# wbw520/scouter

Measured on AMD Instinct MI355X. Metric: images/sec training step (resnest26d+xSlot, 224^2, bs70), higher is better.
Workload: dtype f32; 1 GPU; BASELINE configs[1]: ImageNet-10 resnest26d + positive xSlot, channel 2048, T=3, to_k_layer 3, power 2, 224x224, per-GPU batch 70, random init, AdamW lr 1e-4; precision=fp32, activation_storage=fp32, register_split_bf16x3_layers=16, global_batch=70, parallelism=dp1, step=zero_grad+fwd+loss+bwd(+allreduce)+adamw, launch=eager

## Files before the change

### include/scouter_hip.h

```cpp
#ifndef SCOUTER_HIP_H
#define SCOUTER_HIP_H
#include <stddef.h>
#ifdef __cplusplus
extern "C" {
#endif

#define SC_OK 0
#define SC_ERR_ARG (-1)
#define SC_ERR_LAUNCH (-2)
#define SC_ERR_UNSUPPORTED (-3)
#define SC_ERR_WORKSPACE (-4)

int scouter_abi_version(void);
const char* scouter_last_error(void);

int scouter_set_switch(const char* name, int value);
int scouter_get_switch(const char* name);

int scouter_resize_normalize_u8_f32(const unsigned char* const* srcs, const int* hw, unsigned char* tmp,
                                    const long* tmp_off, const float* lut, float* out, int B, int C, int max_h, int max_w,
                                    int out_h, int out_w, void* stream);

void scouter_prof_enable(int on);
int scouter_prof_collect(char* buf, int cap);
// ... 258 lines not shown

int scouter_linear_small_fwd_f32(const float* x, const float* w, const float* bias, float* y, int B, int K, int C,
                                 void* stream);
int scouter_linear_small_bwd_f32(const float* dy, const float* x, const float* w, float* dx, float* dw, float* db,
                                 int B, int K, int C, void* stream);

int scouter_planes_split_f32(const float* x, void* planes, long n, int nplanes, void* stream);
int scouter_planes_split_weight_f32(const float* w_hwio, void* w_fwd, void* w_dgrad, int kh, int kw, int Cin, int Cout,
                                    int groups, int nplanes, void* stream);
size_t scouter_planes_split_weights_row_bytes(void);
int scouter_planes_split_weights_multi(const void* table, int nrows, long total, int nplanes, void* stream);
int scouter_conv2d_fwd_planes_bn_partial_rows(int B, int H, int W, int kh, int kw, int stride, int pad);
int scouter_conv2d_fwd_planes_io(const void* x_planes, const void* w_planes, const float* bias, const float* addend,
                                 void* y, double* bn_partial, int B, int H, int W, int Cin, int Cout, int kh, int kw,
                                 int stride, int pad, int groups, int relu, int nplanes, int tile, int io, void* stream);
int scouter_conv2d_fwd_planes(const void* x_planes, const void* w_planes, const float* bias, const float* addend,
                              float* y, double* bn_partial, int B, int H, int W, int Cin, int Cout, int kh, int kw,
                              int stride, int pad, int groups, int relu, int nplanes, int tile, void* stream);
int scouter_conv2d_dgrad_planes(const void* dy_planes, const void* w_planes, const float* addend, float* dx, int B, int H,
                                int W, int Cin, int Cout, int kh, int kw, int stride, int pad, int groups, int nplanes,
                                int tile, void* stream);
int scouter_conv2d_dgrad_planes_bnbwd(const void* dy_planes, const void* w_planes, const float* addend, float* dx, int B,
                                      int H, int W, int Cin, int Cout, int kh, int kw, int stride, int pad, int groups,
                                      int nplanes, int tile, const void* relu_mask, const float* x1,
                                      const float* saved1, double* part1, const float* x2, const float* saved2,
                                      double* part2, void* stream);

size_t scouter_conv2d_wgrad_planes_workspace_bytes(int B, int H, int W, int Cin, int Cout, int kh, int kw, int groups,
                                                   int plan_hint);
int scouter_conv2d_wgrad_planes(const void* x_planes, const void* dy_planes, float* dw, int B, int H, int W, int Cin,
                                int Cout, int kh, int kw, int pad, int groups, int nplanes, int plan_hint,
                                void* ws, size_t ws_bytes, void* stream);

int scouter_conv2d_x3_tile(long M, int N, int tile_hint);
int scouter_conv2d_x3_partial_rows(long M, int N, int tile_hint);
int scouter_conv2d_x3_halo_partial_rows(int groups);
int scouter_conv2d_fwd_x3(const float* x, const void* w_planes_fwd, const float* bias, const float* addend, float* y,
                          double* bn_partial, int B, int H, int W, int Cin, int Cout, int kh, int kw, int pad, int groups,
                          int relu, int tile_hint, void* stream);
int scouter_conv2d_dgrad_x3_bnbwd(const float* dy, const void* w_planes_dgrad, const float* addend, float* dx, int B,
                                  int H, int W, int Cin, int Cout, int kh, int kw, int pad, int groups, int tile_hint,
                                  const void* relu_mask, const float* x1, const float* saved1, double* part1,
                                  const float* x2, const float* saved2, double* part2, void* stream);

size_t scouter_conv2d_wgrad_x3_workspace_bytes(int B, int H, int W, int Cin, int Cout, int plan_hint);
int scouter_conv2d_wgrad_x3(const float* x, const float* dy, float* dw, int B, int H, int W, int Cin, int Cout,
                            int plan_hint, void* ws, size_t ws_bytes, void* stream);

size_t scouter_bn_fold_row_bytes(void);
int scouter_bn_fold_multi(const void* table, int nrows, long total, void* stream);
int scouter_sa_gate_fwd_f32(const float* gap, const float* w1, const float* b1, const float* w2, const float* b2, float* a,
                            int B, int Cp, int A, void* stream);

int scouter_iadd_i64(long* p, long n, long v, void* stream);

int scouter_adamw_chunk_bytes(void);
int scouter_adamw_step_f32(const void* chunk_table, int nchunks, const float* grads, float* exp_avg,
                           float* exp_avg_sq, float lr, float beta1, float beta2, float eps, float weight_decay,
                           int step, void* stream);
int scouter_adamw_step_dev_f32(const void* chunk_table, int nchunks, const float* grads, float* exp_avg,
                               float* exp_avg_sq, const float* dyn, float beta1, float beta2, float eps,
                               float weight_decay, void* stream);

#ifdef __cplusplus
}
#endif
#endif
```

### scouter_amd/csrc/abi_core.hip

```cpp
#include "common.h"

#include <stdarg.h>
#include <stdlib.h>
#include <atomic>
#include <map>
#include <mutex>
#include <vector>

#define SCOUTER_ABI_VERSION 1

static thread_local char g_err[512] = "";
static thread_local hipError_t g_lds_err = hipSuccess;

void sc_set_error(const char* fmt, ...) {
    va_list ap;
    va_start(ap, fmt);
    vsnprintf(g_err, sizeof(g_err), fmt, ap);
    va_end(ap);
}

int sc_check_launch(const char* what) {
    hipError_t e = hipGetLastError();
    if (e == hipSuccess) e = g_lds_err;
    g_lds_err = hipSuccess;
    if (e != hipSuccess) {
        sc_set_error("%s: launch failed: %s", what, hipGetErrorString(e));
        return SC_ERR_LAUNCH;
    }
    return SC_OK;
}

extern "C" int scouter_abi_version(void) { return SCOUTER_ABI_VERSION; }
extern "C" const char* scouter_last_error(void) { return g_err; }

static const char* const g_switch_names[SC_SW_COUNT] = {"xwt", "bwt", "bhalo", "xslot_small", "xslot_bwd_halves",
                                                         "xslot_bwd_scratch", "pwp_bn", "pwp_resident"};
struct SwitchTable {
    std::atomic<int> v[SC_SW_COUNT] = {};
    SwitchTable() {
        static const char* const flags[] = {"SCOUTER_XWT", "SCOUTER_BWT", "SCOUTER_BHALO", "SCOUTER_XSLOT_SMALL",
                                            "SCOUTER_XSLOT_BWD_HALVES", "SCOUTER_XSLOT_BWD_SCRATCH"};
        for (int i = 0; i <= SC_SW_XSLOT_BWD_SCRATCH; ++i) {
            const int def = i != SC_SW_XSLOT_BWD_SCRATCH;
            const char* e = getenv(flags[i]);
            v[i] = e && e[0] == '1' - def ? !def : def;
        }
        int bn = 0, r = 0;
        const char* e = getenv("SCOUTER_PWP_PLAN_DEV");
        if (e && sscanf(e, "%d,%d", &bn, &r) == 2 && bn > 0 && r > 0) { v[SC_SW_PWP_BN] = bn; v[SC_SW_PWP_RESIDENT] = r; }
    }
};
static SwitchTable& switch_table() {
    static SwitchTable t;
    return t;
}
int sc_switch(ScSwitch s) { return switch_table().v[s].load(std::memory_order_relaxed); }

static int switch_index(const char* name) {
    for (int i = 0; name && i < SC_SW_COUNT; ++i)
        if (strcmp(name, g_switch_names[i]) == 0) return i;
    sc_set_error("unknown switch '%s'", name ? name : "(null)");
    return -1;
}
extern "C" int scouter_set_switch(const char* name, int value) {
    const int i = switch_index(name);
    if (i < 0) return SC_ERR_ARG;
    SC_REQUIRE(value >= 0, "switch '%s': negative value %d", name, value);
    switch_table().v[i].store(value, std::memory_order_relaxed);
    return SC_OK;
}
extern "C" int scouter_get_switch(const char* name) {
    const int i = switch_index(name);
    return i < 0 ? SC_ERR_ARG : sc_switch((ScSwitch)i);
}

void sc_dyn_lds(const void* kern, size_t bytes) {
    static std::mutex mu;
    static std::map<std::pair<const void*, int>, size_t> limits;
    int dev = 0;
    hipGetDevice(&dev);
    std::lock_guard<std::mutex> lk(mu);
    size_t& have = limits[{kern, dev}];
    if (bytes <= have) return;
    const hipError_t e = hipFuncSetAttribute(kern, hipFuncAttributeMaxDynamicSharedMemorySize, (int)bytes);
    if (e == hipSuccess) have = bytes;
    else g_lds_err = e;
}

struct ProfRec { hipEvent_t a, b; const char* name; double flops, bytes; };
static std::mutex g_prof_mu;
static bool g_prof_on = false;
static std::vector<ProfRec> g_prof;

ScProfScope::ScProfScope(const char* name, hipStream_t st, double flops, double bytes) : stream(st), slot(-1) {
    if (!g_prof_on) return;
// ... 47 lines not shown
```

### scouter_amd/csrc/common.h

```cpp
#pragma once
#include <hip/hip_runtime.h>
#include <stdint.h>
#include <stdio.h>
#include <string.h>

#define SC_OK 0
#define SC_ERR_ARG (-1)
#define SC_ERR_LAUNCH (-2)
#define SC_ERR_UNSUPPORTED (-3)
#define SC_ERR_WORKSPACE (-4)

typedef float f32x4 __attribute__((ext_vector_type(4)));
typedef float f32x16 __attribute__((ext_vector_type(16)));

void sc_set_error(const char* fmt, ...);
int sc_check_launch(const char* what);

enum ScSwitch { SC_SW_XWT, SC_SW_BWT, SC_SW_BHALO, SC_SW_XSLOT_SMALL, SC_SW_XSLOT_BWD_HALVES, SC_SW_XSLOT_BWD_SCRATCH,
                SC_SW_PWP_BN, SC_SW_PWP_RESIDENT, SC_SW_COUNT };
int sc_switch(ScSwitch s);

void sc_dyn_lds(const void* kern, size_t bytes);

#define SC_REQUIRE(cond, ...)                 \
    do {                                      \
        if (!(cond)) {                        \
            sc_set_error(__VA_ARGS__);        \
            return SC_ERR_ARG;                \
        }                                     \
    } while (0)

#define SC_UNSUPPORTED(cond, ...)             \
    do {                                      \
        if (!(cond)) {                        \
            sc_set_error(__VA_ARGS__);        \
            return SC_ERR_UNSUPPORTED;        \
        }                                     \
    } while (0)

struct ScProfScope {
    hipStream_t stream;
    int slot;
    ScProfScope(const char* name, hipStream_t stream, double flops, double bytes);
    ~ScProfScope();
};

static inline int sc_cdiv(long a, long b) { return (int)((a + b - 1) / b); }

__device__ __forceinline__ f32x16 mfma32(float a, float b, f32x16 c) {
    return __builtin_amdgcn_mfma_f32_32x32x2f32(a, b, c, 0, 0, 0);
}
__device__ __forceinline__ int mfma32_row(int reg, int lane) { return (reg & 3) + 8 * (reg >> 2) + 4 * (lane >> 5); }

__device__ __forceinline__ float wave_sum(float v) {
#pragma unroll
    for (int o = 32; o > 0; o >>= 1) v += __shfl_xor(v, o, 64);
    return v;
}
__device__ __forceinline__ double wave_sum_d(double v) {
#pragma unroll
    for (int o = 32; o > 0; o >>= 1) v += __shfl_xor(v, o, 64);
    return v;
}

typedef unsigned short u16x4 __attribute__((ext_vector_type(4)));
__device__ __forceinline__ void split3_bf16(float x, unsigned short& h, unsigned short& m, unsigned short& l) {
    const __bf16 bh = (__bf16)x;
    const float r1 = x - (float)bh;
    const __bf16 bm = (__bf16)r1;
    const float r2 = r1 - (float)bm;
    const __bf16 bl = (__bf16)r2;
    h = __builtin_bit_cast(unsigned short, bh);
// ... 122 lines not shown
```

### scouter_amd/kernels.py

```python
import contextlib
import os
import sys
import types

import torch

from . import _native

F32 = torch.float32
BF16 = torch.bfloat16
IO_X_BF16, IO_Y_BF16, IO_R_BF16 = 1, 2, 4
DGRAD_IO_ADDEND, DGRAD_IO_DY, DGRAD_IO_DX = 4, 8, 16
_ws = {}


_raw_stream = getattr(torch._C, "_cuda_getCurrentRawStream", None)


def _stream():
    if _raw_stream is not None:
        return _raw_stream(torch.cuda.current_device())
    return torch.cuda.current_stream().cuda_stream


# ... 1078 lines not shown
    ws = _sa_ws(B, H * W, C2, x.device)
    _native.check(_native.lib().scouter_sa_reduce_io(_p(x), _p(dout), _p(bn), _p(out), _p(sums), B, H * W, C2 // 2, 1,
                                                     IO_X_BF16 if x.dtype == BF16 else 0, _p(ws), ws.numel(), _stream()),
                  "sa_dattn")
    return (out, sums) if want_stats else out


def sa_bn_bwd(dout, a, dgap, x0, bn, training, dgamma=None, dbeta=None, planes=0, keep_f32=True, sums=None):
    _chk(x0, "x0", (F32, BF16)); _chk(dout, "dout")
    B, H, W, Cp = dout.shape
    dx = torch.empty(x0.shape, dtype=F32, device=x0.device) if keep_f32 or not planes else None
    dxp = torch.empty((planes,) + tuple(x0.shape), dtype=BF16, device=x0.device) if planes else None
    ws = _col_ws(B * H * W, 2 * Cp, x0.device)
    _native.check(_native.lib().scouter_sa_bn_bwd_io(_p(dout), _p(a), _p(dgap), _p(x0), _p(bn), _p(sums), B, H * W, Cp,
                                                     int(training), _p(dgamma), _p(dbeta), _p(dx), _p(dxp), planes,
                                                     IO_X_BF16 if x0.dtype == BF16 else 0, _p(ws), ws.numel(), _stream()),
                  "sa_bn_bwd")
    return PlaneTensor(dx, dxp) if planes else dx


def radix_softmax_fwd(z):
    a = torch.empty_like(z)
    _native.check(_native.lib().scouter_radix_softmax_fwd_f32(_p(z), _p(a), z.shape[0], z.shape[1] // 2, _stream()),
                  "radix_softmax_fwd")
    return a


def radix_softmax_bwd(a, da):
    dz = torch.empty_like(a)
    _native.check(_native.lib().scouter_radix_softmax_bwd_f32(_p(a), _p(da), _p(dz), a.shape[0], a.shape[1] // 2,
                                                              _stream()), "radix_softmax_bwd")
    return dz


SA_GATE_THREADS = 256


def sa_gate_eligible(Cp, A):
    return A in (32, 64, 128, 256) and Cp <= 512 and Cp % (8 * (SA_GATE_THREADS // A)) == 0


def sa_gate_fwd(gap, w1, b1, w2, b2):
    for n, t in (("gap", gap), ("w1", w1), ("b1", b1), ("w2", w2), ("b2", b2)):
        _chk(t, n)
    B, Cp = gap.shape
    A = w1.shape[-1]
    assert tuple(w1.shape[-2:]) == (Cp, A) and tuple(w2.shape[-2:]) == (A, 2 * Cp) and b1.numel() == A and b2.numel() == 2 * Cp
    a = torch.empty((B, 2 * Cp), dtype=F32, device=gap.device)
    _native.check(_native.lib().scouter_sa_gate_fwd_f32(_p(gap), _p(w1), _p(b1), _p(w2), _p(b2), _p(a), B, Cp, A, _stream()),
                  "sa_gate_fwd")
    return a


class BnFolder:

    def __init__(self, items):
        import struct
        L = _native.lib()
        dev = items[0][0].device
        self.key = self.pointers(items)
        if any(it[0].data_ptr() % 16 for it in items):
            raise RuntimeError("scouter_amd: the one-launch fold reads the weights as 16-byte vectors: unaligned weight storage")
        al = lambda n: (n + 63) // 64 * 64
        offs, off = [], 0
        for w, cb, g, be, mu, var, eps, rows_pad in items:
            cout = w.shape[-1]
            rows = w.numel() // cout
            if cout % 4 or rows_pad and rows_pad < rows:
                raise RuntimeError("scouter_amd: the one-launch fold takes 4-multiples of output channels, got %s" % (tuple(w.shape),))
            offs.append((off, off + al(max(rows, rows_pad) * cout)))
            off = offs[-1][1] + al(cout)
        self.flat = torch.zeros(off, dtype=F32, device=dev)
        rows_blob, self.outs, first = [], [], 0
        for (w, cb, g, be, mu, var, eps, rows_pad), (ow, ob) in zip(items, offs):
            for n, t in (("weight", w), ("conv bias", cb), ("gamma", g), ("beta", be), ("running_mean", mu), ("running_var", var)):
                _chk(t, n)
            cout = w.shape[-1]
            rows = w.numel() // cout
            shape = (1, 1, rows_pad, cout) if rows_pad else tuple(w.shape)
            wo = self.flat[ow:ow + max(rows, rows_pad) * cout].view(shape)
            bo = self.flat[ob:ob + cout]
            rows_blob.append(struct.pack("<6Qd2Qiiq", w.data_ptr(), _p(cb) or 0, g.data_ptr(), be.data_ptr(), mu.data_ptr(),
                                         var.data_ptr(), float(eps), wo.data_ptr(), bo.data_ptr(), rows, cout, first))
            self.outs.append((wo, bo))
            first += rows * cout
        blob = b"".join(rows_blob)
        assert len(blob) == len(items) * L.scouter_bn_fold_row_bytes()
        self.table = torch.frombuffer(bytearray(blob), dtype=torch.uint8).to(dev)
        self.total = first

    @staticmethod
    def pointers(items):
        return tuple(t.data_ptr() if t is not None else 0 for it in items for t in it[:6])

    def run(self):
        _native.check(_native.lib().scouter_bn_fold_multi(_p(self.table), len(self.outs), self.total, _stream()), "bn_fold_multi")
        return self.outs


def sa_apply_fwd(x, a, bn=None, out_dtype=F32):
    _chk(x, "x", (F32, BF16))
    B, H, W, C2 = x.shape
    out = torch.empty((B, H, W, C2 // 2), dtype=out_dtype, device=x.device)
    _native.check(_native.lib().scouter_sa_apply_fwd_io(
        _p(x), _p(a), _p(bn), _p(out), B, H * W, C2 // 2,
        (IO_X_BF16 if x.dtype == BF16 else 0) | (IO_Y_BF16 if out_dtype == BF16 else 0), _stream()), "sa_apply_fwd")
# ... 696 lines not shown
```

### scouter_amd/timm/models/layers/split_attn.py

```python
import os

import torch.nn as nn

from ....nn_hip import Act, BatchNorm2d, Conv2d
from .... import kernels as K

SA_SUMS = os.environ.get("SCOUTER_SA_SUMS", "1") == "1"


class SplitAttnConv2d(nn.Module):
    def __init__(self, in_channels, out_channels, kernel_size=3, stride=1, padding=1, groups=1, radix=2,
                 reduction_factor=4):
        super().__init__()
        if radix != 2 or groups != 1:
            raise NotImplementedError("scouter_amd supports the radix-2 / cardinality-1 split attention of "
                                      "resnest26d / resnest50d only")
        self.radix = radix
        mid_chs = out_channels * radix
        attn_chs = max(in_channels * radix // reduction_factor, 32)
        self.conv = Conv2d(in_channels, mid_chs, kernel_size, stride, padding, groups=groups * radix, bias=False)
        self.bn0 = BatchNorm2d(mid_chs)
        self.act0 = Act()
        self.fc1 = Conv2d(out_channels, attn_chs, 1, bias=True)
        self.bn1 = BatchNorm2d(attn_chs)
        self.act1 = Act()
        self.fc2 = Conv2d(attn_chs, mid_chs, 1, bias=True)

    def fwd(self, x, save, tracked=None, x0_dtype=None, out_dtype=None):
        c, c_conv = self.conv.fwd(x, save, bn_stats=self.bn0.training, out_dtype=x0_dtype)
        x0, saved0 = self.bn0.stats_only(c, tracked)
        B = x0.shape[0]
        gap = K.sa_gap(x0, saved0)
        z1, c_fc1 = self.fc1.fwd(gap.view(B, 1, 1, -1), save, bn_stats=self.bn1.training)
        g1, c_bn1 = self.bn1.fwd(z1, save, relu=True, tracked=tracked)
        z2, c_fc2 = self.fc2.fwd(g1, save)
        a = K.radix_softmax_fwd(z2.view(B, -1))
        out = K.sa_apply_fwd(x0, a, saved0, out_dtype=out_dtype or K.F32)
        return out, ((c_conv, x0, saved0, self.bn0.training, c_fc1, c_bn1, c_fc2, a) if save else None)

    def fwd_folded(self, x):
        x0 = self.conv.fwd_folded(x, relu=True)
        B = x0.shape[0]
        gap = K.sa_gap(x0, None)
        if K.sa_gate_eligible(gap.shape[1], self.fc1.out_channels):
            f = self.fc1._fold
            a = K.sa_gate_fwd(gap, f.w, f.b, K.hwio(self.fc2.weight), self.fc2.bias)
        else:
            g1 = self.fc1.fwd_folded(gap.view(B, 1, 1, -1), relu=True)
            z2, _ = self.fc2.fwd(g1, False)
            a = K.radix_softmax_fwd(z2.view(B, -1))
        return K.sa_apply_fwd(x0, a, None)

    def bwd(self, dout, ctx, post=None):
        c_conv, x0, saved0, training0, c_fc1, c_bn1, c_fc2, a = ctx
        B = x0.shape[0]
        da, sums = K.sa_dattn(x0, dout, saved0, want_stats=True) if SA_SUMS else (K.sa_dattn(x0, dout, saved0), None)
        dz2 = K.radix_softmax_bwd(a, da)
        dg1 = self.fc2.bwd(dz2.view(B, 1, 1, -1), c_fc2, True)
        dz1, _ = self.bn1.bwd(dg1, c_bn1)
        dgap = self.fc1.bwd(dz1, c_fc1, True)
        on_planes = c_conv.wd is not None
        only = on_planes and c_conv.xp is not None and self.conv.planes_only(x0.shape[1], x0.shape[2])
        planes = self.conv.route().planes_dy if on_planes else 0
        if not planes and self.conv.dy_plane_only(*x0.shape[:3]):
            planes, only = 1, True
        dc = K.sa_bn_bwd(dout, a, dgap.view(B, -1), x0, saved0, training0, self.bn0._dg, self.bn0._db,
                         planes=planes, keep_f32=not only, sums=sums)
        return self.conv.bwd(dc, c_conv, True, post=post)
```

Before: 4819 images/sec.

## Fuse split-attention gate fc1+BN+ReLU, fc2+softmax and backward into custom kernels

Adds dedicated HIP kernels for the split-attention gate in training: fc1 with batch-norm stats and ReLU, fc2 with radix softmax, a fused softmax-backward/fc2-dgrad/BN-backward kernel, an fc1 dgrad kernel, and a combined weight-gradient kernel that runs on a side stream. The aim is to replace a chain of many small launches (conv, BN, softmax, colsum) on tiny B x C tensors with a few launches. The path is gated by a new default-on switch and a shape eligibility check. The trade-off is added code complexity and a different numerical path for BN statistics, which are accumulated in double.

```diff
diff --git a/include/scouter_hip.h b/include/scouter_hip.h
--- a/include/scouter_hip.h
+++ b/include/scouter_hip.h
@@ -334,6 +334,20 @@
 int scouter_sa_gate_fwd_f32(const float* gap, const float* w1, const float* b1, const float* w2, const float* b2, float* a,
                             int B, int Cp, int A, void* stream);
 
+int scouter_sa_gate_train_ok(int B, int Cp, int A);
+int scouter_sa_gate_train_max_batch(void);
+int scouter_sa_gate_fc1_bn_f32(const float* gap, const float* w1, const float* b1, const float* gamma, const float* beta,
+                               float* running_mean, float* running_var, float momentum, float eps, float* z1, float* g1,
+                               float* saved, int B, int Cp, int A, void* stream);
+int scouter_sa_gate_fc2_softmax_f32(const float* g1, const float* w2, const float* b2, float* a, int B, int Cp, int A,
+                                    void* stream);
+int scouter_sa_gate_bwd_fc2_bn_f32(const float* a, const float* da, const float* w2, const float* g1, const float* z1,
+                                   const float* gamma, float eps, float* dz2, float* dz1, float* dgamma, float* dbeta, int B,
+                                   int Cp, int A, void* stream);
+int scouter_sa_gate_bwd_fc1_f32(const float* dz1, const float* w1, float* dgap, int B, int Cp, int A, void* stream);
+int scouter_sa_gate_wgrad_f32(const float* gap, const float* dz1, const float* g1, const float* dz2, float* dw1, float* db1,
+                              float* dw2, float* db2, int B, int Cp, int A, void* stream);
+
 int scouter_iadd_i64(long* p, long n, long v, void* stream);
 
 int scouter_adamw_chunk_bytes(void);
diff --git a/scouter_amd/csrc/abi_core.hip b/scouter_amd/csrc/abi_core.hip
--- a/scouter_amd/csrc/abi_core.hip
+++ b/scouter_amd/csrc/abi_core.hip
@@ -34,13 +34,13 @@
 extern "C" const char* scouter_last_error(void) { return g_err; }
 
 static const char* const g_switch_names[SC_SW_COUNT] = {"xwt", "bwt", "bhalo", "xslot_small", "xslot_bwd_halves",
-                                                         "xslot_bwd_scratch", "pwp_bn", "pwp_resident"};
+                                                         "xslot_bwd_scratch", "sa_gate_train", "pwp_bn", "pwp_resident"};
 struct SwitchTable {
     std::atomic<int> v[SC_SW_COUNT] = {};
     SwitchTable() {
         static const char* const flags[] = {"SCOUTER_XWT", "SCOUTER_BWT", "SCOUTER_BHALO", "SCOUTER_XSLOT_SMALL",
-                                            "SCOUTER_XSLOT_BWD_HALVES", "SCOUTER_XSLOT_BWD_SCRATCH"};
-        for (int i = 0; i <= SC_SW_XSLOT_BWD_SCRATCH; ++i) {
+                                            "SCOUTER_XSLOT_BWD_HALVES", "SCOUTER_XSLOT_BWD_SCRATCH", "SCOUTER_SA_GATE_TRAIN"};
+        for (int i = 0; i <= SC_SW_SA_GATE_TRAIN; ++i) {
             const int def = i != SC_SW_XSLOT_BWD_SCRATCH;
             const char* e = getenv(flags[i]);
             v[i] = e && e[0] == '1' - def ? !def : def;
diff --git a/scouter_amd/csrc/common.h b/scouter_amd/csrc/common.h
--- a/scouter_amd/csrc/common.h
+++ b/scouter_amd/csrc/common.h
@@ -17,7 +17,7 @@
 int sc_check_launch(const char* what);
 
 enum ScSwitch { SC_SW_XWT, SC_SW_BWT, SC_SW_BHALO, SC_SW_XSLOT_SMALL, SC_SW_XSLOT_BWD_HALVES, SC_SW_XSLOT_BWD_SCRATCH,
-                SC_SW_PWP_BN, SC_SW_PWP_RESIDENT, SC_SW_COUNT };
+                SC_SW_SA_GATE_TRAIN, SC_SW_PWP_BN, SC_SW_PWP_RESIDENT, SC_SW_COUNT };
 int sc_switch(ScSwitch s);
 
 void sc_dyn_lds(const void* kern, size_t bytes);
diff --git a/scouter_amd/csrc/sa_gate_train.hip b/scouter_amd/csrc/sa_gate_train.hip
--- /dev/null
+++ b/scouter_amd/csrc/sa_gate_train.hip
@@ -0,0 +1,391 @@
+#include "common.h"
+
+#define SGT_THREADS 256
+#define SGT_MAX_B 256
+#define SGT_MAX_CP 512
+#define SGT_MAX_A 256
+#define SGT_NC 8
+#ifndef SGT_FC1_ACC
+#define SGT_FC1_ACC double
+#endif
+
+static bool sgt_shape_ok(long B, long Cp, long A) {
+    return (A == 32 || A == 64 || A == 128 || A == 256) && Cp >= 32 && Cp <= SGT_MAX_CP && Cp % 32 == 0 && B >= 2 &&
+           B <= SGT_MAX_B;
+}
+extern "C" int scouter_sa_gate_train_ok(int B, int Cp, int A) { return sgt_shape_ok(B, Cp, A) ? 1 : 0; }
+extern "C" int scouter_sa_gate_train_max_batch(void) { return SGT_MAX_B; }
+
+template <int NC>
+__device__ __forceinline__ int sgt_wrow(int k) { return k * NC + (k >> 2) * 4; }
+
+__device__ __forceinline__ float sgt_fma(float a, float b, float c) { return __builtin_fmaf(a, b, c); }
+__device__ __forceinline__ double sgt_fma(double a, double b, double c) { return __builtin_fma(a, b, c); }
+
+template <int NC, typename T>
+__device__ __forceinline__ void sgt_tile_dot(const float* __restrict__ xrow, int K, const float* ws, int ks, T (&acc)[NC]) {
+#pragma unroll
+    for (int j = 0; j < NC; ++j) acc[j] = 0;
+    if (xrow) {
+#pragma unroll 4
+        for (int k0 = 4 * ks; k0 < K; k0 += 32) {
+            const f32x4 x = *(const f32x4*)(xrow + k0);
+#pragma unroll
+            for (int u = 0; u < 4; ++u) {
+                const float* w = ws + (k0 + u) * NC + k0;
+#pragma unroll
+                for (int j = 0; j < NC; j += 4) {
+                    const f32x4 wv = *(const f32x4*)(w + j);
+#pragma unroll
+                    for (int q = 0; q < 4; ++q) acc[j + q] = sgt_fma((T)x[u], (T)wv[q], acc[j + q]);
+                }
+            }
+        }
+    }
+#pragma unroll
+    for (int o = 1; o < 8; o <<= 1)
+#pragma unroll
+        for (int j = 0; j < NC; ++j) acc[j] += __shfl_xor(acc[j], o, 64);
+}
+
+__global__ __launch_bounds__(SGT_THREADS) void gate_fc1_bn_kernel(
+    const float* __restrict__ gap, const float* __restrict__ w1, const float* __restrict__ b1, const float* __restrict__ gamma,
+    const float* __restrict__ beta, float* __restrict__ rmean, float* __restrict__ rvar, float momentum, float eps,
+    float* __restrict__ z1, float* __restrict__ g1, float* __restrict__ saved, int B, int Cp, int A) {
+    __shared__ float ws[SGT_MAX_CP * (SGT_NC + 1)];
+    __shared__ float zs[SGT_MAX_B * SGT_NC];
+    __shared__ double red[32][SGT_NC][2];
+    __shared__ float par[3][SGT_NC];
+    const int tid = threadIdx.x, j0 = blockIdx.x * SGT_NC;
+    for (int i = tid; i < Cp * 2; i += SGT_THREADS) {
+        const int k = i >> 1, h = (i & 1) * 4;
+        *(f32x4*)(ws + sgt_wrow<SGT_NC>(k) + h) = *(const f32x4*)(w1 + (long)k * A + j0 + h);
+    }
+    __syncthreads();
+    const int ks = tid & 7, r = tid >> 3;
+    const f32x4 blo = *(const f32x4*)(b1 + j0), bhi = *(const f32x4*)(b1 + j0 + 4);
+    for (int b0 = 0; b0 < B; b0 += 32) {
+        const int b = b0 + r;
+        SGT_FC1_ACC acc[SGT_NC];
+        sgt_tile_dot<SGT_NC>(b < B ? gap + (long)b * Cp : nullptr, Cp, ws, ks, acc);
+        if (b < B && ks == 0) {
+#pragma unroll
+            for (int h = 0; h < 2; ++h) {
+                const f32x4 bias = h ? bhi : blo;
+                f32x4 z;
+#pragma unroll
+                for (int k = 0; k < 4; ++k) z[k] = (float)(acc[4 * h + k] + (SGT_FC1_ACC)bias[k]);
+                *(f32x4*)(zs + b * SGT_NC + 4 * h) = z;
+            }
+        }
+    }
+    __syncthreads();
+    {
+        const int j = tid & 7, p = tid >> 3;
+        double s = 0, t = 0;
+        for (int b = p; b < B; b += 32) {
+            const double v = zs[b * SGT_NC + j];
+            s += v; t += v * v;
+        }
+        red[p][j][0] = s; red[p][j][1] = t;
+    }
+    __syncthreads();
+    if (tid < SGT_NC) {
+        const int c = j0 + tid;
+        double s = 0, t = 0;
+        for (int p = 0; p < 32; ++p) { s += red[p][tid][0]; t += red[p][tid][1]; }
+        const double mean = s / (double)B;
+        double var = t / (double)B - mean * mean;
+        if (var < 0) var = 0;
+        const double unb = var * (double)B / (double)(B - 1);
+        rmean[c] = (float)((1.0 - momentum) * rmean[c] + momentum * mean);
+        rvar[c] = (float)((1.0 - momentum) * rvar[c] + momentum * unb);
+        const float rstd = (float)(1.0 / sqrt(var + (double)eps));
+        const float sc = gamma[c] * rstd, sh = beta[c];
+        saved[c] = (float)mean; saved[A + c] = rstd; saved[2 * A + c] = sc; saved[3 * A + c] = sh;
+        par[0][tid] = (float)mean; par[1][tid] = sc; par[2][tid] = sh;
+    }
+    __syncthreads();
+    for (int i = tid; i < B * 2; i += SGT_THREADS) {
+        const int b = i >> 1, h = (i & 1) * 4;
+        const f32x4 z = *(const f32x4*)(zs + b * SGT_NC + h);
+        f32x4 g;
+#pragma unroll
+        for (int k = 0; k < 4; ++k) g[k] = fmaxf(fmaf(z[k] - par[0][h + k], par[1][h + k], par[2][h + k]), 0.f);
+        *(f32x4*)(z1 + (long)b * A + j0 + h) = z;
+        *(f32x4*)(g1 + (long)b * A + j0 + h) = g;
+    }
+}
+
+__global__ __launch_bounds__(SGT_THREADS) void gate_fc2_softmax_kernel(const float* __restrict__ g1, const float* __restrict__ w2,
+                                                                       const float* __restrict__ b2, float* __restrict__ a, int B,
+                                                                       int Cp, int A) {
+    __shared__ float ws[SGT_MAX_A * (2 * SGT_NC + 1)];
+    const int tid = threadIdx.x, c0 = blockIdx.x * SGT_NC, C2 = 2 * Cp;
+    for (int i = tid; i < A * 4; i += SGT_THREADS) {
+        const int k = i >> 2, q = i & 3;
+        const int col = q < 2 ? c0 + 4 * q : Cp + c0 + 4 * (q - 2);
+        *(f32x4*)(ws + sgt_wrow<2 * SGT_NC>(k) + 4 * q) = *(const f32x4*)(w2 + (long)k * C2 + col);
+    }
+    __syncthreads();
+    const int ks = tid & 7, r = tid >> 3;
+    const float bias0 = b2[c0 + ks], bias1 = b2[Cp + c0 + ks];
+    const int b_end = min(B, (int)(blockIdx.y + 1) * 64);
+    for (int b0 = blockIdx.y * 64; b0 < b_end; b0 += 32) {
+        const int b = b0 + r;
+        float acc[2 * SGT_NC];
+        sgt_tile_dot<2 * SGT_NC>(b < B ? g1 + (long)b * A : nullptr, A, ws, ks, acc);
+        float z0 = acc[0], z1 = acc[SGT_NC];
+#pragma unroll
+        for (int j = 1; j < SGT_NC; ++j) { z0 = ks == j ? acc[j] : z0; z1 = ks == j ? acc[SGT_NC + j] : z1; }
+        if (b < B) {
+            z0 += bias0; z1 += bias1;
+            const float m = fmaxf(z0, z1), e0 = expf(z0 - m), e1 = expf(z1 - m), inv = 1.f / (e0 + e1);
+            a[(long)b * C2 + c0 + ks] = e0 * inv;
+            a[(long)b * C2 + Cp + c0 + ks] = e1 * inv;
+        }
+    }
+}
+
+__global__ __launch_bounds__(SGT_THREADS) void gate_bwd_fc2_bn_kernel(
+    const float* __restrict__ a, const float* __restrict__ da, const float* __restrict__ w2, const float* __restrict__ g1,
+    const float* __restrict__ z1, const float* __restrict__ gamma, float eps, float* __restrict__ dz2,
+    float* __restrict__ dz1, float* __restrict__ dgamma, float* __restrict__ dbeta, int B, int Cp, int A) {
+    __shared__ float ws[2 * SGT_MAX_CP * (SGT_NC + 1)];
+    __shared__ float gs[SGT_MAX_B * SGT_NC];
+    __shared__ double red[32][SGT_NC][2];
+    __shared__ double coef[2][SGT_NC];
+    const int tid = threadIdx.x, j0 = blockIdx.x * SGT_NC, C2 = 2 * Cp, q4 = C2 >> 2;
+    for (int i = tid; i < SGT_NC * q4; i += SGT_THREADS) {
+        const int n = i / q4, k = (i % q4) * 4;
+        const f32x4 w = *(const f32x4*)(w2 + (long)(j0 + n) * C2 + k);
+#pragma unroll
+        for (int u = 0; u < 4; ++u) ws[(k + u) * SGT_NC + k + n] = w[u];
+    }
+    __syncthreads();
+    const int ks = tid & 7, r = tid >> 3;
+    for (int b0 = 0; b0 < B; b0 += 32) {
+        const int b = b0 + r;
+        float acc[SGT_NC];
+#pragma unroll
+        for (int j = 0; j < SGT_NC; ++j) acc[j] = 0.f;
+        if (b < B) {
+            const long row = (long)b * C2;
+#pragma unroll 2
+            for (int k0 = 4 * ks; k0 < Cp; k0 += 32) {
+                const f32x4 a0 = *(const f32x4*)(a + row + k0), a1 = *(const f32x4*)(a + row + Cp + k0);
+                const f32x4 d0 = *(const f32x4*)(da + row + k0), d1 = *(const f32x4*)(da + row + Cp + k0);
+                f32x4 y0, y1;
+#pragma unroll
+                for (int u = 0; u < 4; ++u) {
+                    const float dot = a0[u] * d0[u] + a1[u] * d1[u];
+                    y0[u] = a0[u] * (d0[u] - dot);
+                    y1[u] = a1[u] * (d1[u] - dot);
+                }
+                if ((k0 >> 5) % (int)gridDim.x == (int)blockIdx.x) {
+                    *(f32x4*)(dz2 + row + k0) = y0;
+                    *(f32x4*)(dz2 + row + Cp + k0) = y1;
+                }
+#pragma unroll
+                for (int u = 0; u < 4; ++u) {
+                    const float* wa = ws + (k0 + u) * SGT_NC + k0;
+                    const float* wb = ws + (Cp + k0 + u) * SGT_NC + Cp + k0;
+#pragma unroll
+                    for (int j = 0; j < SGT_NC; j += 4) {
+                        const f32x4 va = *(const f32x4*)(wa + j), vb = *(const f32x4*)(wb + j);
+#pragma unroll
+                        for (int q = 0; q < 4; ++q)
+                            acc[j + q] = __builtin_fmaf(y1[u], vb[q], __builtin_fmaf(y0[u], va[q], acc[j + q]));
+                    }
+                }
+            }
+        }
+#pragma unroll
+        for (int o = 1; o < 8; o <<= 1)
+#pragma unroll
+            for (int j = 0; j < SGT_NC; ++j) acc[j] += __shfl_xor(acc[j], o, 64);
+        if (b < B && ks == 0) {
+            const f32x4 ylo = *(const f32x4*)(g1 + (long)b * A + j0), yhi = *(const f32x4*)(g1 + (long)b * A + j0 + 4);
+            *(f32x4*)(gs + b * SGT_NC) = f32x4{ylo[0] > 0.f ? acc[0] : 0.f, ylo[1] > 0.f ? acc[1] : 0.f,
+                                               ylo[2] > 0.f ? acc[2] : 0.f, ylo[3] > 0.f ? acc[3] : 0.f};
+            *(f32x4*)(gs + b * SGT_NC + 4) = f32x4{yhi[0] > 0.f ? acc[4] : 0.f, yhi[1] > 0.f ? acc[5] : 0.f,
+                                                   yhi[2] > 0.f ? acc[6] : 0.f, yhi[3] > 0.f ? acc[7] : 0.f};
+        }
+    }
+    __syncthreads();
+    const int j = tid & 7, p = tid >> 3;
+    {
+        double s = 0, t = 0;
+        for (int b = p; b < B; b += 32) {
+            const double v = z1[(long)b * A + j0 + j];
+            s += v; t += v * v;
+        }
+        red[p][j][0] = s; red[p][j][1] = t;
+    }
+    __syncthreads();
+    if (tid < SGT_NC) {
+        double s = 0, t = 0;
+        for (int q = 0; q < 32; ++q) { s += red[q][tid][0]; t += red[q][tid][1]; }
+        const double mean = s / (double)B;
+        double var = t / (double)B - mean * mean;
+        if (var < 0) var = 0;
+        coef[0][tid] = mean;
+        coef[1][tid] = 1.0 / sqrt(var + (double)eps);
+    }
+    __syncthreads();
+    const double mu = coef[0][j], rs = coef[1][j], sc = (double)gamma[j0 + j] * rs;
+    __syncthreads();
+    {
+        double s = 0, t = 0;
+        for (int b = p; b < B; b += 32) {
+            const double g = gs[b * SGT_NC + j];
+            s += g; t += g * (((double)z1[(long)b * A + j0 + j] - mu) * rs);
+        }
+        red[p][j][0] = s; red[p][j][1] = t;
+    }
+    __syncthreads();
+    if (tid < SGT_NC) {
+        double s = 0, t = 0;
+        for (int q = 0; q < 32; ++q) { s += red[q][tid][0]; t += red[q][tid][1]; }
+        if (dbeta) dbeta[j0 + tid] = (float)s;
+        if (dgamma) dgamma[j0 + tid] = (float)t;
+        coef[0][tid] = s / (double)B;
+        coef[1][tid] = t / (double)B;
+    }
+    __syncthreads();
+    const double k1 = coef[0][j], k2 = coef[1][j];
+    for (int b = p; b < B; b += 32) {
+        const double xh = ((double)z1[(long)b * A + j0 + j] - mu) * rs;
+        dz1[(long)b * A + j0 + j] = (float)(sc * ((double)gs[b * SGT_NC + j] - k1 - xh * k2));
+    }
+}
+
+__global__ __launch_bounds__(SGT_THREADS) void gate_bwd_fc1_kernel(const float* __restrict__ dz1, const float* __restrict__ w1,
+                                                                   float* __restrict__ dgap, int B, int Cp, int A) {
+    __shared__ float ws[SGT_MAX_A * (SGT_NC + 1)];
+    const int tid = threadIdx.x, c0 = blockIdx.x * SGT_NC, q4 = A >> 2;
+    for (int i = tid; i < SGT_NC * q4; i += SGT_THREADS) {
+        const int n = i / q4, k = (i % q4) * 4;
+        const f32x4 w = *(const f32x4*)(w1 + (long)(c0 + n) * A + k);
+#pragma unroll
+        for (int u = 0; u < 4; ++u) ws[(k + u) * SGT_NC + k + n] = w[u];
+    }
+    __syncthreads();
+    const int ks = tid & 7, r = tid >> 3;
+    const int b_end = min(B, (int)(blockIdx.y + 1) * 64);
+    for (int b0 = blockIdx.y * 64; b0 < b_end; b0 += 32) {
+        const int b = b0 + r;
+        float acc[SGT_NC];
+        sgt_tile_dot<SGT_NC>(b < B ? dz1 + (long)b * A : nullptr, A, ws, ks, acc);
+        const f32x4 o = ks ? f32x4{acc[4], acc[5], acc[6], acc[7]} : f32x4{acc[0], acc[1], acc[2], acc[3]};
+        if (b < B && ks < 2) *(f32x4*)(dgap + (long)b * Cp + c0 + 4 * ks) = o;
+    }
+}
+
+__global__ __launch_bounds__(SGT_THREADS) void gate_wgrad_kernel(const float* __restrict__ gap, const float* __restrict__ dz1,
+                                                                 const float* __restrict__ g1, const float* __restrict__ dz2,
+                                                                 float* __restrict__ dw1, float* __restrict__ db1,
+                                                                 float* __restrict__ dw2, float* __restrict__ db2, int B, int Cp,
+                                                                 int A, int n1) {
+    __shared__ float xs[32 * 32];
+    __shared__ float ys[32 * 32];
+    int t = blockIdx.x;
+    const bool first = t < n1;
+    if (!first) t -= n1;
+    const float* X = first ? gap : g1;
+    const float* Y = first ? dz1 : dz2;
+    float* dw = first ? dw1 : dw2;
+    float* db = first ? db1 : db2;
+    const int R = first ? Cp : A, C = first ? A : 2 * Cp;
+    const int ct = C >> 5, r0 = (t / ct) * 32, c0 = (t % ct) * 32;
+    const int tid = threadIdx.x, r = tid >> 3, cq = (tid & 7) * 4;
+    const bool bias = db != nullptr && r0 == 0 && r == 0;
+    float acc[4] = {0.f, 0.f, 0.f, 0.f};
+    double bs[4] = {0, 0, 0, 0};
+    for (int b0 = 0; b0 < B; b0 += 32) {
+        const int b = b0 + r;
+        f32x4 xv = {0.f, 0.f, 0.f, 0.f}, yv = {0.f, 0.f, 0.f, 0.f};
+        if (b < B) {
+            xv = *(const f32x4*)(X + (long)b * R + r0 + cq);
+            yv = *(const f32x4*)(Y + (long)b * C + c0 + cq);
+        }
+        *(f32x4*)(xs + r * 32 + cq) = xv;
+        *(f32x4*)(ys + r * 32 + cq) = yv;
+        __syncthreads();
+#pragma unroll 8
+        for (int i = 0; i < 32; ++i) {
+            const float x = xs[i * 32 + r];
+            const f32x4 y = *(const f32x4*)(ys + i * 32 + cq);
+#pragma unroll
+            for (int k = 0; k < 4; ++k) acc[k] = __builtin_fmaf(x, y[k], acc[k]);
+            if (bias) {
+#pragma unroll
+                for (int k = 0; k < 4; ++k) bs[k] += (double)y[k];
+            }
+        }
+        __syncthreads();
+    }
+    if (dw) *(f32x4*)(dw + (long)(r0 + r) * C + c0 + cq) = f32x4{acc[0], acc[1], acc[2], acc[3]};
+    if (bias) *(f32x4*)(db + c0 + cq) = f32x4{(float)bs[0], (float)bs[1], (float)bs[2], (float)bs[3]};
+}
+
+#define SGT_SHAPE(what)                                                                                                          \
+    SC_REQUIRE(B > 0 && Cp > 0 && A > 0, what ": empty shape");                                                                  \
+    SC_UNSUPPORTED(sgt_shape_ok(B, Cp, A),                                                                                       \
+                   what ": covers attention widths 32 / 64 / 128 / 256, 32-multiples of channels up to %d and 2 to %d rows "     \
+                        "(got B %d, Cp %d, width %d)", SGT_MAX_CP, SGT_MAX_B, B, Cp, A)
+
+extern "C" int scouter_sa_gate_fc1_bn_f32(const float* gap, const float* w1, const float* b1, const float* gamma,
+                                          const float* beta, float* running_mean, float* running_var, float momentum, float eps,
+                                          float* z1, float* g1, float* saved, int B, int Cp, int A, void* stream) {
+    SC_REQUIRE(gap && w1 && b1 && gamma && beta && running_mean && running_var && z1 && g1 && saved,
+               "sa_gate_fc1_bn: null pointer");
+    SGT_SHAPE("sa_gate_fc1_bn");
+    ScProfScope prof("sa_gate_fc1_bn", (hipStream_t)stream, 2.0 * B * Cp * A, 4.0 * (B * Cp + Cp * A + 2.0 * B * A));
+    hipLaunchKernelGGL(gate_fc1_bn_kernel, dim3(A / SGT_NC), dim3(SGT_THREADS), 0, (hipStream_t)stream, gap, w1, b1, gamma, beta,
+                       running_mean, running_var, momentum, eps, z1, g1, saved, B, Cp, A);
+    return sc_check_launch("sa_gate_fc1_bn");
+}
+
+extern "C" int scouter_sa_gate_fc2_softmax_f32(const float* g1, const float* w2, const float* b2, float* a, int B, int Cp, int A,
+                                               void* stream) {
+    SC_REQUIRE(g1 && w2 && b2 && a, "sa_gate_fc2_softmax: null pointer");
+    SGT_SHAPE("sa_gate_fc2_softmax");
+    ScProfScope prof("sa_gate_fc2_softmax", (hipStream_t)stream, 4.0 * B * Cp * A, 4.0 * (B * A + 2.0 * Cp * A + 2.0 * B * Cp));
+    hipLaunchKernelGGL(gate_fc2_softmax_kernel, dim3(Cp / SGT_NC, sc_cdiv(B, 64)), dim3(SGT_THREADS), 0, (hipStream_t)stream, g1,
+                       w2, b2, a, B, Cp, A);
+    return sc_check_launch("sa_gate_fc2_softmax");
+}
+
+extern "C" int scouter_sa_gate_bwd_fc2_bn_f32(const float* a, const float* da, const float* w2, const float* g1, const float* z1,
+                                              const float* gamma, float eps, float* dz2, float* dz1, float* dgamma, float* dbeta,
+                                              int B, int Cp, int A, void* stream) {
+    SC_REQUIRE(a && da && w2 && g1 && z1 && gamma && dz2 && dz1, "sa_gate_bwd_fc2_bn: null pointer");
+    SGT_SHAPE("sa_gate_bwd_fc2_bn");
+    ScProfScope prof("sa_gate_bwd_fc2_bn", (hipStream_t)stream, 4.0 * B * Cp * A, 4.0 * (6.0 * B * Cp + 2.0 * Cp * A + 3.0 * B * A));
+    hipLaunchKernelGGL(gate_bwd_fc2_bn_kernel, dim3(A / SGT_NC), dim3(SGT_THREADS), 0, (hipStream_t)stream, a, da, w2, g1, z1,
+                       gamma, eps, dz2, dz1, dgamma, dbeta, B, Cp, A);
+    return sc_check_launch("sa_gate_bwd_fc2_bn");
+}
+
+extern "C" int scouter_sa_gate_bwd_fc1_f32(const float* dz1, const float* w1, float* dgap, int B, int Cp, int A, void* stream) {
+    SC_REQUIRE(dz1 && w1 && dgap, "sa_gate_bwd_fc1: null pointer");
+    SGT_SHAPE("sa_gate_bwd_fc1");
+    ScProfScope prof("sa_gate_bwd_fc1", (hipStream_t)stream, 2.0 * B * Cp * A, 4.0 * (B * A + Cp * A + (double)B * Cp));
+    hipLaunchKernelGGL(gate_bwd_fc1_kernel, dim3(Cp / SGT_NC, sc_cdiv(B, 64)), dim3(SGT_THREADS), 0, (hipStream_t)stream, dz1, w1,
+                       dgap, B, Cp, A);
+    return sc_check_launch("sa_gate_bwd_fc1");
+}
+
+extern "C" int scouter_sa_gate_wgrad_f32(const float* gap, const float* dz1, const float* g1, const float* dz2, float* dw1,
+                                         float* db1, float* dw2, float* db2, int B, int Cp, int A, void* stream) {
+    SC_REQUIRE(gap && dz1 && g1 && dz2, "sa_gate_wgrad: null pointer");
+    SGT_SHAPE("sa_gate_wgrad");
+    const int n1 = dw1 ? (Cp / 32) * (A / 32) : db1 ? A / 32 : 0;
+    const int n2 = dw2 ? (A / 32) * (2 * Cp / 32) : db2 ? 2 * Cp / 32 : 0;
+    if (n1 + n2 == 0) return SC_OK;
+    ScProfScope prof("sa_gate_wgrad", (hipStream_t)stream, 6.0 * B * Cp * A, 4.0 * (3.0 * B * Cp + 2.0 * B * A + 3.0 * Cp * A));
+    hipLaunchKernelGGL(gate_wgrad_kernel, dim3(n1 + n2), dim3(SGT_THREADS), 0, (hipStream_t)stream, gap, dz1, g1, dz2, dw1, db1,
+                       dw2, db2, B, Cp, A, n1);
+    return sc_check_launch("sa_gate_wgrad");
+}
diff --git a/scouter_amd/kernels.py b/scouter_amd/kernels.py
--- a/scouter_amd/kernels.py
+++ b/scouter_amd/kernels.py
@@ -1154,6 +1154,84 @@
     return a
 
 
+_sa_gate_train_asked = {}
+
+
+def sa_gate_train_eligible(B, Cp, A):
+    key = (B, Cp, A)
+    v = _sa_gate_train_asked.get(key)
+    if v is None:
+        v = _sa_gate_train_asked[key] = bool(_native.lib().scouter_sa_gate_train_ok(B, Cp, A))
+    return v
+
+
+def sa_gate_train_max_batch():
+    return _native.lib().scouter_sa_gate_train_max_batch()
+
+
+def sa_gate_fc1_bn(gap, w1, b1, gamma, beta, running_mean, running_var, momentum=0.1, eps=1e-5):
+    for n, t in (("gap", gap), ("w1", w1), ("b1", b1), ("gamma", gamma), ("beta", beta), ("running_mean", running_mean),
+                 ("running_var", running_var)):
+        _chk(t, n)
+    B, Cp = gap.shape
+    A = w1.shape[-1]
+    assert tuple(w1.shape[-2:]) == (Cp, A) and b1.numel() == A and gamma.numel() == A and running_mean.numel() == A
+    z1 = torch.empty((B, A), dtype=F32, device=gap.device)
+    g1 = torch.empty((B, A), dtype=F32, device=gap.device)
+    saved = torch.empty((4, A), dtype=F32, device=gap.device)
+    _native.check(_native.lib().scouter_sa_gate_fc1_bn_f32(_p(gap), _p(w1), _p(b1), _p(gamma), _p(beta), _p(running_mean),
+                                                           _p(running_var), momentum, eps, _p(z1), _p(g1), _p(saved), B, Cp, A,
+                                                           _stream()), "sa_gate_fc1_bn")
+    return z1, g1, saved
+
+
+def sa_gate_fc2_softmax(g1, w2, b2):
+    _chk(g1, "g1"); _chk(w2, "w2"); _chk(b2, "b2")
+    B, A = g1.shape
+    C2 = w2.shape[-1]
+    assert tuple(w2.shape[-2:]) == (A, C2) and b2.numel() == C2
+    a = torch.empty((B, C2), dtype=F32, device=g1.device)
+    _native.check(_native.lib().scouter_sa_gate_fc2_softmax_f32(_p(g1), _p(w2), _p(b2), _p(a), B, C2 // 2, A, _stream()),
+                  "sa_gate_fc2_softmax")
+    return a
+
+
+def sa_gate_bwd_fc2_bn(a, da, w2, g1, z1, gamma, dgamma=None, dbeta=None, eps=1e-5):
+    for n, t in (("a", a), ("da", da), ("w2", w2), ("g1", g1), ("z1", z1), ("gamma", gamma)):
+        _chk(t, n)
+    B, A = g1.shape
+    C2 = a.shape[1]
+    assert tuple(w2.shape[-2:]) == (A, C2) and da.shape == a.shape and z1.shape == g1.shape and gamma.numel() == A
+    dz2 = torch.empty_like(a)
+    dz1 = torch.empty_like(g1)
+    _native.check(_native.lib().scouter_sa_gate_bwd_fc2_bn_f32(_p(a), _p(da), _p(w2), _p(g1), _p(z1), _p(gamma), eps, _p(dz2),
+                                                               _p(dz1), _p(dgamma), _p(dbeta), B, C2 // 2, A, _stream()),
+                  "sa_gate_bwd_fc2_bn")
+    return dz2, dz1
+
+
+def sa_gate_bwd_fc1(dz1, w1):
+    _chk(dz1, "dz1"); _chk(w1, "w1")
+    B, A = dz1.shape
+    Cp = w1.shape[-2]
+    assert w1.shape[-1] == A
+    dgap = torch.empty((B, Cp), dtype=F32, device=dz1.device)
+    _native.check(_native.lib().scouter_sa_gate_bwd_fc1_f32(_p(dz1), _p(w1), _p(dgap), B, Cp, A, _stream()), "sa_gate_bwd_fc1")
+    return dgap
+
+
+def sa_gate_wgrad(gap, dz1, g1, dz2, dw1=None, db1=None, dw2=None, db2=None):
+    for n, t in (("gap", gap), ("dz1", dz1), ("g1", g1), ("dz2", dz2), ("dw1", dw1), ("db1", db1), ("dw2", dw2), ("db2", db2)):
+        _chk(t, n)
+    B, Cp = gap.shape
+    A = g1.shape[1]
+    assert dz1.shape == g1.shape and tuple(dz2.shape) == (B, 2 * Cp)
+    assert dw1 is None or dw1.numel() == Cp * A
+    assert dw2 is None or dw2.numel() == 2 * Cp * A
+    _native.check(_native.lib().scouter_sa_gate_wgrad_f32(_p(gap), _p(dz1), _p(g1), _p(dz2), _p(dw1), _p(db1), _p(dw2), _p(db2),
+                                                          B, Cp, A, _stream()), "sa_gate_wgrad")
+
+
 class BnFolder:
 
     def __init__(self, items):
diff --git a/scouter_amd/timm/models/layers/split_attn.py b/scouter_amd/timm/models/layers/split_attn.py
--- a/scouter_amd/timm/models/layers/split_attn.py
+++ b/scouter_amd/timm/models/layers/split_attn.py
@@ -1,4 +1,5 @@
 import os
+from collections import namedtuple
 
 import torch.nn as nn
 
@@ -6,6 +7,7 @@
 from .... import kernels as K
 
 SA_SUMS = os.environ.get("SCOUTER_SA_SUMS", "1") == "1"
+GateCtx = namedtuple("GateCtx", "gap z1 g1")
 
 
 class SplitAttnConv2d(nn.Module):
@@ -31,12 +33,37 @@
         x0, saved0 = self.bn0.stats_only(c, tracked)
         B = x0.shape[0]
         gap = K.sa_gap(x0, saved0)
-        z1, c_fc1 = self.fc1.fwd(gap.view(B, 1, 1, -1), save, bn_stats=self.bn1.training)
-        g1, c_bn1 = self.bn1.fwd(z1, save, relu=True, tracked=tracked)
-        z2, c_fc2 = self.fc2.fwd(g1, save)
-        a = K.radix_softmax_fwd(z2.view(B, -1))
+        if self._gate_fused(B):
+            bn1 = self.bn1
+            z1, g1, _ = K.sa_gate_fc1_bn(gap, K.hwio(self.fc1.weight), self.fc1.bias, bn1.weight, bn1.bias,
+                                         bn1.running_mean, bn1.running_var, bn1.momentum, bn1.eps)
+            if tracked is not None:
+                tracked.append(bn1.num_batches_tracked)
+            if bn1._capture is not None:
+                bn1._capture[0][bn1._capture[1]] = g1.view(B, 1, 1, -1)
+            a = K.sa_gate_fc2_softmax(g1, K.hwio(self.fc2.weight), self.fc2.bias)
+            c_fc1, c_bn1, c_fc2 = GateCtx(gap, z1, g1), None, None
+        else:
+            z1, c_fc1 = self.fc1.fwd(gap.view(B, 1, 1, -1), save, bn_stats=self.bn1.training)
+            g1, c_bn1 = self.bn1.fwd(z1, save, relu=True, tracked=tracked)
+            z2, c_fc2 = self.fc2.fwd(g1, save)
+            a = K.radix_softmax_fwd(z2.view(B, -1))
         out = K.sa_apply_fwd(x0, a, saved0, out_dtype=out_dtype or K.F32)
         return out, ((c_conv, x0, saved0, self.bn0.training, c_fc1, c_bn1, c_fc2, a) if save else None)
+
+    def _gate_fused(self, B):
+        return bool(self.bn1.training and K.get_switch("sa_gate_train") and
+                    K.sa_gate_train_eligible(B, self.fc1.in_channels, self.fc1.out_channels))
+
+    def _gate_bwd(self, da, a, g):
+        fc1, fc2, bn1 = self.fc1, self.fc2, self.bn1
+        dz2, dz1 = K.sa_gate_bwd_fc2_bn(a, da, K.hwio(fc2.weight), g.g1, g.z1, bn1.weight, bn1._dg, bn1._db,
+                                          bn1.eps)
+        dgap = K.sa_gate_bwd_fc1(dz1, K.hwio(fc1.weight))
+        if any(t is not None for t in (fc1._dw, fc1._db, fc2._dw, fc2._db)):
+            with K.side_stream(da.device, g.gap, dz1, g.g1, dz2, enabled=fc1.use_side_stream):
+                K.sa_gate_wgrad(g.gap, dz1, g.g1, dz2, fc1._dw, fc1._db, fc2._dw, fc2._db)
+        return dgap
 
     def fwd_folded(self, x):
         x0 = self.conv.fwd_folded(x, relu=True)
@@ -55,10 +82,13 @@
         c_conv, x0, saved0, training0, c_fc1, c_bn1, c_fc2, a = ctx
         B = x0.shape[0]
         da, sums = K.sa_dattn(x0, dout, saved0, want_stats=True) if SA_SUMS else (K.sa_dattn(x0, dout, saved0), None)
-        dz2 = K.radix_softmax_bwd(a, da)
-        dg1 = self.fc2.bwd(dz2.view(B, 1, 1, -1), c_fc2, True)
-        dz1, _ = self.bn1.bwd(dg1, c_bn1)
-        dgap = self.fc1.bwd(dz1, c_fc1, True)
+        if isinstance(c_fc1, GateCtx):
+            dgap = self._gate_bwd(da, a, c_fc1)
+        else:
+            dz2 = K.radix_softmax_bwd(a, da)
+            dg1 = self.fc2.bwd(dz2.view(B, 1, 1, -1), c_fc2, True)
+            dz1, _ = self.bn1.bwd(dg1, c_bn1)
+            dgap = self.fc1.bwd(dz1, c_fc1, True)
         on_planes = c_conv.wd is not None
         only = on_planes and c_conv.xp is not None and self.conv.planes_only(x0.shape[1], x0.shape[2])
         planes = self.conv.route().planes_dy if on_planes else 0
diff --git a/tools_dev/sa_gate_bench.py b/tools_dev/sa_gate_bench.py
--- /dev/null
+++ b/tools_dev/sa_gate_bench.py
@@ -0,0 +1,169 @@
+import argparse
+import contextlib
+import os
+import sys
+
+import torch
+import torch.nn as nn
+
+sys.path.insert(0, os.path.dirname(os.path.dirname(os.path.abspath(__file__))))
+
+import __graft_entry__ as G
+
+G.build()
+from scouter_amd import kernels as K
+from scouter_amd.nn_hip import BatchNorm2d, Conv2d, GradArena
+
+SHAPES = ((64, 32), (128, 64), (256, 128), (512, 256))
+LEGS = ("forward", "backward main", "backward side")
+
+
+class Gate(nn.Module):
+    def __init__(self, Cp, A):
+        super().__init__()
+        self.fc1, self.bn1, self.fc2 = Conv2d(Cp, A, 1, bias=True), BatchNorm2d(A), Conv2d(A, 2 * Cp, 1, bias=True)
+
+
+@contextlib.contextmanager
+def no_param_grads(*convs):
+    kept = [(c, c._dw, c._db) for c in convs]
+    for c in convs:
+        c._dw = c._db = None
+    try:
+        yield
+    finally:
+        for c, dw, db in kept:
+            c._dw, c._db = dw, db
+
+
+def legs(Cp, A, B):
+    m = Gate(Cp, A).cuda().train()
+    GradArena(m)
+    fc1, bn1, fc2 = m.fc1, m.bn1, m.fc2
+    fc1.use_side_stream = fc2.use_side_stream = False
+    g = torch.Generator().manual_seed(Cp + B)
+    gap = (torch.randn(B, Cp, generator=g).abs() * 0.6).cuda()
+    da = (torch.randn(B, 2 * Cp, generator=g) * 0.1).cuda()
+    gap4 = gap.view(B, 1, 1, Cp)
+    w1, w2 = K.hwio(fc1.weight), K.hwio(fc2.weight)
+    st = {}
+
+    def old_fwd():
+        z1, c1 = fc1.fwd(gap4, True, bn_stats=True)
+        g1, cb = bn1.fwd(z1, True, relu=True)
+        z2, c2 = fc2.fwd(g1, True)
+        st["old"] = (c1, cb, c2, K.radix_softmax_fwd(z2.view(B, -1)), g1)
+
+    def new_fwd():
+        z1, g1, saved = K.sa_gate_fc1_bn(gap, w1, fc1.bias, bn1.weight, bn1.bias, bn1.running_mean, bn1.running_var)
+        st["new"] = (z1, g1, saved, K.sa_gate_fc2_softmax(g1, w2, fc2.bias))
+
+    def old_main():
+        c1, cb, c2, a, g1 = st["old"]
+        with no_param_grads(fc1, fc2):
+            dz2 = K.radix_softmax_bwd(a, da)
+            dg1 = fc2.bwd(dz2.view(B, 1, 1, -1), c2, True)
+            dz1, _ = bn1.bwd(dg1, cb)
+            fc1.bwd(dz1, c1, True)
+        st["old_b"] = (dz1, dz2)
+
+    def new_main():
+        z1, g1, saved, a = st["new"]
+        dz2, dz1 = K.sa_gate_bwd_fc2_bn(a, da, w2, g1, z1, bn1.weight, bn1._dg, bn1._db)
+        K.sa_gate_bwd_fc1(dz1, w1)
+        st["new_b"] = (dz1, dz2)
+
+    def old_side():
+        dz1, dz2 = st["old_b"]
+        g1 = st["old"][4]
+        K.conv2d_wgrad(gap4, dz1, fc1._dw)
+        K.colsum(dz1, fc1._db)
+        K.conv2d_wgrad(g1, dz2.view(B, 1, 1, -1), fc2._dw)
+        K.colsum(dz2, fc2._db)
+
+    def new_side():
+        dz1, dz2 = st["new_b"]
+        K.sa_gate_wgrad(gap, dz1, st["new"][1], dz2, fc1._dw, fc1._db, fc2._dw, fc2._db)
+
+    return {"forward": (old_fwd, new_fwd), "backward main": (old_main, new_main), "backward side": (old_side, new_side)}
+
+
+def graph_us(fn, passes=20, replays=10):
+    s = torch.cuda.Stream()
+    s.wait_stream(torch.cuda.current_stream())
+    with torch.cuda.stream(s):
+        fn()
+        fn()
+    torch.cuda.current_stream().wait_stream(s)
+    torch.cuda.synchronize()
+    graph = torch.cuda.CUDAGraph()
+    with torch.cuda.graph(graph):
+        for _ in range(passes):
+            fn()
+    graph.replay()
+    torch.cuda.synchronize()
+    e0, e1 = torch.cuda.Event(enable_timing=True), torch.cuda.Event(enable_timing=True)
+    e0.record()
+    for _ in range(replays):
+        graph.replay()
+    e1.record()
+    torch.cuda.synchronize()
+    return e0.elapsed_time(e1) * 1e3 / (passes * replays)
+
+
+def eager_us(fn, passes=200):
+    for _ in range(5):
+        fn()
+    torch.cuda.synchronize()
+    e0, e1 = torch.cuda.Event(enable_timing=True), torch.cuda.Event(enable_timing=True)
+    e0.record()
+    for _ in range(passes):
+        fn()
+    e1.record()
+    torch.cuda.synchronize()
+    return e0.elapsed_time(e1) * 1e3 / passes
+
+
+def main():
+    ap = argparse.ArgumentParser()
+    ap.add_argument("--batch", type=int, default=70)
+    ap.add_argument("--repeats", type=int, default=3)
+    ap.add_argument("--out", default=None)
+    a = ap.parse_args()
+    lines = []
+
+    def say(s):
+        print(s, flush=True)
+        lines.append(s)
+
+    med = lambda v: sorted(v)[len(v) // 2]
+    fmt = lambda v: " ".join("%.1f" % t for t in v)
+    total = {(leg, r, k): 0.0 for leg in LEGS for r in ("old", "new") for k in ("graph", "eager")}
+    say("split-attention gate, training, B = %d: us per pass (graph replay | eager), %d alternating repeats" % (a.batch, a.repeats))
+    for Cp, A in SHAPES:
+        L = legs(Cp, A, a.batch)
+        for leg in LEGS:
+            t = {(r, k): [] for r in ("old", "new") for k in ("graph", "eager")}
+            for _ in range(a.repeats):
+                for r, fn in zip(("old", "new"), L[leg]):
+                    t[(r, "graph")].append(graph_us(fn))
+                    t[(r, "eager")].append(eager_us(fn))
+            say("(%3d, %3d) %-14s old: graph %s | eager %s    new: graph %s | eager %s    graph old / new %.2f"
+                % (Cp, A, leg, fmt(t[("old", "graph")]), fmt(t[("old", "eager")]), fmt(t[("new", "graph")]),
+                   fmt(t[("new", "eager")]), med(t[("old", "graph")]) / med(t[("new", "graph")])))
+            for key, v in t.items():
+                total[(leg,) + key] += 2 * med(v)
+    for leg in LEGS:
+        say("8 blocks, %-14s old: graph %.0f us, eager %.0f us    new: graph %.0f us, eager %.0f us"
+            % (leg, total[(leg, "old", "graph")], total[(leg, "old", "eager")], total[(leg, "new", "graph")],
+               total[(leg, "new", "eager")]))
+    for r in ("old", "new"):
+        say("8 blocks, all legs, %s: graph %.0f us, eager %.0f us"
+            % (r, sum(total[(leg, r, "graph")] for leg in LEGS), sum(total[(leg, r, "eager")] for leg in LEGS)))
+    if a.out:
+        with open(a.out, "w") as f:
+            f.write("\n".join(lines) + "\n")
+
+
+if __name__ == "__main__":
+    main()
```

Result: no change. 4855 images/sec, median of 6 (+0.8%).
